# awslabs/flowgger

Measured on NVIDIA H100. Metric: log lines/sec parsed (RFC5424), higher is better.
Workload: dtype u8

## Files before the change

### flowgger_b200/csrc/fg_abi.cu

```cuda
#include <cuda_runtime.h>

#include <algorithm>
#include <chrono>
#include <cstdio>
#include <cstdlib>
#include <cstring>
#include <ctime>
#include <mutex>
#include <new>
#include <string>
#include <utility>
#include <vector>

#include "../../include/flowgger_cuda.h"
#include "fg_kernels.cuh"
#include "fg_status.h"
#include "fg_rfc3164.cuh"
#include "fg_tz.h"

namespace {

const char* kErrorStrings[FG_ST_COUNT] = {};
struct ErrorTableInit {
    ErrorTableInit() {
// ... 301 lines not shown
    int upload(fg_ctx* c, Buf<uint8_t>& blob) {
        bytes.resize(bytes.size() + 16, 0);
        FG_CUDA(c, blob.alloc(bytes.size(), DEV));
        FG_CUDA(c, cudaMemcpy(blob.d, bytes.data(), bytes.size(), cudaMemcpyHostToDevice));
        return FG_OK;
    }
};

int upload_tz(fg_ctx* c) {
    const fg::TzHostTable& H = c->tz_host;
    Packer p;
    const size_t o_hash = p.add(H.hash), o_key = p.add(H.key), o_zone = p.add(H.zone), o_noff = p.add(H.name_off),
                 o_first = p.add(H.first), o_off = p.add(H.off), o_names = p.add(H.names);
    if (int rc = p.upload(c, c->tz_blob)) return rc;
    const uint8_t* b = c->tz_blob.d;
    fg::TzDeviceTable& T = c->tz_dev;
    T = H.view();
    T.hash = (const unsigned long long*)(b + o_hash);
    T.key = (const long long*)(b + o_key);
    T.zone = (const int32_t*)(b + o_zone);
    T.name_off = (const int32_t*)(b + o_noff);
    T.first = (const int32_t*)(b + o_first);
    T.off = (const int32_t*)(b + o_off);
    T.names = b + o_names;
    return FG_OK;
}

int upload_ltsv_config(fg_ctx* c, const fg_config* cfg) {
    std::vector<uint8_t> names, suffix;
    std::vector<int32_t> name_off{0}, types;
    const int ns = (cfg->ltsv_schema_names && cfg->ltsv_schema_types) ? cfg->ltsv_schema_len : 0;
    for (int k = 0; k < ns; ++k) {
        const char* s = cfg->ltsv_schema_names[k];
        names.insert(names.end(), (const uint8_t*)s, (const uint8_t*)s + strlen(s));
        name_off.push_back((int32_t)names.size());
        types.push_back(cfg->ltsv_schema_types[k]);
    }
    fg::LtsvDeviceConfig& L = c->ltsv;
    L.has_schema = (cfg->ltsv_has_schema || ns > 0) ? 1 : 0;
    L.n_schema = ns;
    L.suffix_present = 0;
    L.suffix_off[0] = 0;
    for (int t = 0; t < 5; ++t) {
        const char* s = cfg->ltsv_suffix[t];
        if (t > 0 && s) {
            L.suffix_present |= 1u << t;
            suffix.insert(suffix.end(), (const uint8_t*)s, (const uint8_t*)s + strlen(s));
        }
        L.suffix_off[t + 1] = (int32_t)suffix.size();
    }
    Packer p;
    const size_t o_names = p.add(names), o_off = p.add(name_off), o_types = p.add(types), o_suf = p.add(suffix);
    if (int rc = p.upload(c, c->ltsv_blob)) return rc;
    const uint8_t* b = c->ltsv_blob.d;
    L.names = b + o_names;
    L.name_off = (const int32_t*)(b + o_off);
    L.types = (const int32_t*)(b + o_types);
    L.suffix = b + o_suf;
    return FG_OK;
}

int current_year(const fg_ctx* c) {
    if (c->r3164_year != 0) return c->r3164_year;
    const time_t now = time(nullptr);
    struct tm g;
    gmtime_r(&now, &g);
    return g.tm_year + 1900;
}

int ensure_format(fg_ctx* c, int fmt) {
    const size_t L = (size_t)c->max_lines;
    if (fmt == FG_FMT_RFC5424) {
        if (!c->rows5.d) {
            FG_CUDA(c, c->rows5.alloc(L, BOTH));
            FG_CUDA(c, c->esc_list.alloc(L, DEV));
            FG_CUDA(c, c->wide_list.alloc(L, DEV));
        }
    } else if (!c->rows.d) {
        FG_CUDA(c, c->rows.alloc(col_off(c, C_COUNT), BOTH));
    }
    if (fmt == FG_FMT_GELF && !c->wide_list.d) FG_CUDA(c, c->wide_list.alloc(L, DEV));
    for (const TableUse& u : kFormatTables[fmt]) {
        const size_t first = u.div ? std::max<size_t>(c->max_bytes / u.div, u.floor) : u.floor;
        const size_t cap = c->tab[u.table].cap;
        if (u.grow ? cap < first : !cap)
            if (int rc = grow_table(c, u.table, first)) return rc;
    }
    if (fmt == FG_FMT_RFC3164) {
        if (!c->tz_host.loaded) {
            std::string err;
            if (!fg::tz_load_dir(c->tzdir.empty() ? nullptr : c->tzdir.c_str(), c->tz_host, err)) return fail(c, FG_E_ARG, err.c_str());
        }
        if (!c->tz_blob.d)
            if (int rc = upload_tz(c)) return rc;
    }
    if (fmt == FG_FMT_LTSV || fmt == FG_FMT_GELF) {
        const size_t need = (fmt == FG_FMT_LTSV ? c->max_bytes / 2 + L : c->max_bytes / 3) + 64;
        if (c->tmp_meta.n < need) {
            c->tmp_name.reset(); c->tmp_val.reset(); c->tmp_meta.reset();
            FG_CUDA(c, c->tmp_name.alloc(need, DEV));
            FG_CUDA(c, c->tmp_val.alloc(need, DEV));
            FG_CUDA(c, c->tmp_meta.alloc(need, DEV));
        }
    }
    return FG_OK;
}

int begin_call(fg_ctx* c, fg_format fmt) {
    if ((int)fmt < 0 || (int)fmt > 3) return fail(c, FG_E_ARG, "unknown format");
    FG_CUDA(c, cudaSetDevice(c->device));
    if (int rc = ensure_format(c, (int)fmt)) return rc;
    c->call_year = current_year(c);
    return FG_OK;
}

int pick_tile(const fg_ctx* c, size_t total_bytes, int n, int fmt) {
    const double mean = n > 0 ? (double)total_bytes / n : 0.0;
    const long lines = fg::lines_per_cta(fmt), gran = 8 * lines;
    const int max_tile[4] = {c->max_tile5, fg::kLtsvMaxTile, fg::kGelfMaxTile, fg::kR3164MaxTile};
    long t = (long)(mean * lines * 1.02) + gran;
    t = (t + gran - 1) / gran * gran;
    t = std::max(t, 8L * 1024);
    t = std::min(t, (long)max_tile[fmt]);
    return (int)t;
}

int launch_lines(fg_ctx* c, int fmt, int line0, int n, int tile, const uint8_t* invalid, int strip_eol, cudaStream_t s,
                 bool time_dominant = false) {
    if (fmt == FG_FMT_RFC5424) {
        fg::Parse5424Params P;
        P.bytes = c->bytes.d;
        P.offsets = c->offsets.d + line0;
        P.n = n;
        P.tile_bytes = tile;
        P.rows = reinterpret_cast<uint4*>(c->rows5.d + line0);
        P.entries = dev<unsigned long long>(c, T_E8);
        P.entry_cap = cap32(c, T_E8);
        P.counters = c->k.d;
        P.esc_list = c->esc_list.d;
        P.wide_list = c->wide_list.d;
        P.arena = dev<uint8_t>(c, T_ARENA);
        P.arena_cap = cap32(c, T_ARENA);
        P.wide_rows = dev<fg::WideRow>(c, T_WIDE);
        P.wide_cap = cap32(c, T_WIDE);
        P.wentry_name = dev<int2>(c, T_ENTRIES, 0);
        P.wentry_val = dev<unsigned long long>(c, T_ENTRIES, 1);
        P.wentry_meta = dev<uint8_t>(c, T_ENTRIES, 2);
        P.wentry_cap = cap32(c, T_ENTRIES);
        P.line0 = line0;
        P.bad_offsets = c->k.d + fg::K5_BAD_OFFSETS;
        P.line_invalid = invalid;
        P.strip_eol = strip_eol;
        P.num_sms = c->num_sms;
        FG_CUDA(c, cudaMemsetAsync(c->k.d + fg::K5_ESC_LIST, 0, 8, s));
        FG_CUDA(c, fg::launch_parse5424(P, s, time_dominant ? c->ev_dom0.h : nullptr, time_dominant ? c->ev_dom1.h : nullptr));
        c->launches += 2;
        return FG_OK;
    }
    fg::ParseParams P;
    P.bytes = c->bytes.d;
    P.offsets = c->offsets.d + line0;
    P.n = n;
    P.line0 = line0;
    P.tile_bytes = tile;
    P.num_sms = c->num_sms;
    uint8_t* r = c->rows.d;
    P.ts = (double*)(r + col_off(c, C_TS)) + line0;
    P.meta = (uint32_t*)(r + col_off(c, C_META)) + line0;
    P.host = (int2*)(r + col_off(c, C_HOST)) + line0;
    P.app = (int2*)(r + col_off(c, C_APP)) + line0;
    P.proc = (int2*)(r + col_off(c, C_PROC)) + line0;
    P.msgid = (int2*)(r + col_off(c, C_MSGID)) + line0;
    P.msg = (int2*)(r + col_off(c, C_MSG)) + line0;
    P.full = (int2*)(r + col_off(c, C_FULL)) + line0;
    P.sd = (int2*)(r + col_off(c, C_SD)) + line0;
    P.entry_name = dev<int2>(c, T_ENTRIES, 0);
    P.entry_val = dev<unsigned long long>(c, T_ENTRIES, 1);
    P.entry_meta = dev<uint8_t>(c, T_ENTRIES, 2);
    P.tmp_name = c->tmp_name.d;
    P.tmp_val = c->tmp_val.d;
    P.tmp_meta = c->tmp_meta.d;
    P.line_invalid = invalid;
    P.strip_eol = strip_eol;
    P.entry_counter = c->k.d + fg::K5_ENTRIES;
    P.entry_cap = cap32(c, T_ENTRIES);
    P.bad_offsets = c->k.d + fg::K5_BAD_OFFSETS;
    P.slow_list = c->wide_list.d;
    P.slow_count = c->k.d + fg::K5_WIDE_LIST;
    if (fmt == FG_FMT_GELF) FG_CUDA(c, cudaMemsetAsync(c->k.d + fg::K5_WIDE_LIST, 0, 4, s));
    P.ltsv = c->ltsv;
    P.r3164.year = c->call_year;
    P.r3164.tz = c->tz_dev;
    P.r3164.arena = dev<uint8_t>(c, T_ARENA);
    P.r3164.arena_cap = cap32(c, T_ARENA);
    P.r3164.arena_counter = c->k.d + fg::K5_ARENA;
    if (time_dominant) FG_CUDA(c, cudaEventRecord(c->ev_dom0, s));
    FG_CUDA(c, fg::launch_parse(fmt, P, s));
    if (time_dominant) FG_CUDA(c, cudaEventRecord(c->ev_dom1, s));
    c->launches += fmt == FG_FMT_GELF ? 2 : 1;
    return FG_OK;
}

bool gelf_fusable(int fmt) { return fmt == FG_FMT_RFC5424 || fmt == FG_FMT_RFC3164; }

int launch_encode(fg_ctx* c, int fmt, int k, int l0, int n, int tile, cudaStream_t s) {
    fg::GelfEncodeParams E{};
    E.bytes = c->bytes.d;
    E.offsets = c->offsets.d + l0;
    E.n = n;
    if (fmt == FG_FMT_RFC5424) {
        E.rows = reinterpret_cast<const uint4*>(c->rows5.d + l0);
    } else {
        const uint8_t* r = c->rows.d;
        E.r3_ts = (const double*)(r + col_off(c, C_TS)) + l0;
        E.r3_meta = (const uint32_t*)(r + col_off(c, C_META)) + l0;
        E.r3_host = (const int2*)(r + col_off(c, C_HOST)) + l0;
        E.r3_msg = (const int2*)(r + col_off(c, C_MSG)) + l0;
        E.r3_full = (const int2*)(r + col_off(c, C_FULL)) + l0;
    }
    E.entries = dev<unsigned long long>(c, T_E8);
    E.arena = dev<uint8_t>(c, T_ARENA);
    E.wide_rows = dev<fg::WideRow>(c, T_WIDE);
    E.wentry_name = dev<int2>(c, T_ENTRIES, 0);
    E.wentry_val = dev<unsigned long long>(c, T_ENTRIES, 1);
    E.wentry_meta = dev<uint8_t>(c, T_ENTRIES, 2);
    E.static_blob = c->static_blob.d;
    E.n_static = c->n_static;
    E.static_key_off = c->d_static_key_off;
    E.static_lit_off = c->d_static_lit_off;
    E.static_kind = c->d_static_kind;
    E.lens = c->enc_lens.d + l0;
    E.rel = c->enc_rel.d + l0;
    E.base = c->enc_base.d + k;
    E.out = c->enc_out.d;
    E.out_cap = c->enc_out_cap;
    E.out_offsets = c->enc_offsets.d + l0;
    E.status = c->enc_status.d + l0;
    E.bad_offsets = c->k.d + fg::K5_BAD_OFFSETS;
    E.entry_cap = cap32(c, T_E8);
    E.wide_cap = cap32(c, T_WIDE);
    E.wentry_cap = cap32(c, T_ENTRIES);
    E.arena_cap = cap32(c, T_ARENA);
    E.tile_bytes = std::min(4 * tile, c->max_tile5);
    FG_CUDA(c, fg::launch_gelf_encode(fmt, E, c->scan_temp.d, c->scan_temp_bytes, s));
    c->launches += 4;
    return FG_OK;
}

bool col_used(int col) { return !(col == C_APP || col == C_PROC || col == C_MSGID); }

void fill_out(fg_ctx* c, int fmt, int n, const uint32_t* tot, fg_batch_out* out) {
    out->n = n;
    for (const TableUse& u : kFormatTables[fmt]) {
        const uint32_t rows = u.counter >= 0 ? tot[u.counter] : 0;
        switch (u.table) {
            case T_ENTRIES:
                out->entry_name = host<fg_span>(c, T_ENTRIES, 0);
                out->entry_val = host<uint64_t>(c, T_ENTRIES, 1);
                out->entry_meta = host<uint8_t>(c, T_ENTRIES, 2);
                out->n_entries = (int32_t)rows;
                break;
            case T_E8:
                out->entries8 = host<uint64_t>(c, T_E8);
                out->n_entries8 = (int32_t)rows;
                break;
            case T_ARENA:
                out->arena = host<uint8_t>(c, T_ARENA);
                out->arena_bytes = (int64_t)rows;
                break;
            case T_WIDE:
                out->wide_rows = host<fg_wide_row>(c, T_WIDE);
                out->n_wide = (int32_t)rows;
                break;
        }
    }
    if (fmt == FG_FMT_RFC5424) {
        out->rows5424 = c->rows5.h;
        return;
    }
    uint8_t* r = c->rows.h;
    out->ts = (const double*)(r + col_off(c, C_TS));
    out->meta = (const uint32_t*)(r + col_off(c, C_META));
    out->hostname = (const fg_span*)(r + col_off(c, C_HOST));
    out->msg = (const fg_span*)(r + col_off(c, C_MSG));
    out->full_msg = (const fg_span*)(r + col_off(c, C_FULL));
    out->sd = (const fg_span*)(r + col_off(c, C_SD));
}

int copy_rows_d2h(fg_ctx* c, int fmt, int line0, int n, cudaStream_t s) {
    if (n <= 0) return FG_OK;
    if (fmt == FG_FMT_RFC5424) {
        FG_CUDA(c, cudaMemcpyAsync(c->rows5.h + line0, c->rows5.d + line0, (size_t)n * 32, cudaMemcpyDeviceToHost, s));
        return FG_OK;
    }
    for (int col = C_TS; col <= C_META; ++col) {
        const size_t o = col_off(c, col) + (size_t)line0 * kColW[col];
        FG_CUDA(c, cudaMemcpyAsync(c->rows.h + o, c->rows.d + o, (size_t)n * kColW[col], cudaMemcpyDeviceToHost, s));
    }
    const size_t pitch = (size_t)c->max_lines * 8;
    int col = C_HOST;
    while (col < C_COUNT) {
        if (!col_used(col)) { ++col; continue; }
        int end = col;
        while (end + 1 < C_COUNT && col_used(end + 1)) ++end;
        const size_t o = col_off(c, col) + (size_t)line0 * 8;
        FG_CUDA(c, cudaMemcpy2DAsync(c->rows.h + o, pitch, c->rows.d + o, pitch, (size_t)n * 8, (size_t)(end - col + 1),
                                     cudaMemcpyDeviceToHost, s));
// ... 762 lines not shown
```

### flowgger_b200/csrc/fg_kernels.cuh

```cuda
#pragma once
#include <stdint.h>
#ifdef FG_HOST_EMU
#include "../../tests/emu/cuda_shim.h"
#else
#include <cuda_runtime.h>
#endif

namespace fg {

struct LtsvDeviceConfig {
    int32_t has_schema;
    int32_t n_schema;
    const uint8_t* names;
    const int32_t* name_off;
    const int32_t* types;
    const uint8_t* suffix;
    int32_t suffix_off[6];
    uint32_t suffix_present;
};

struct TzDeviceTable {
    int32_t n_names;
    int32_t min_len, max_len;
    uint32_t first_mask[8];
    const unsigned long long* hash;
    const int32_t* zone;
    const int32_t* name_off;
    const uint8_t* names;
    const int32_t* first;
    const long long* key;
    const int32_t* off;
};
struct R3164DeviceConfig {
    int32_t year;
    TzDeviceTable tz;
    uint8_t* arena;
    uint32_t arena_cap;
    uint32_t* arena_counter;
};

struct ParseParams {
    const uint8_t* bytes;
    const int32_t* offsets;
    int32_t n;
    int32_t line0;
    int32_t tile_bytes;
    double* ts;
    uint32_t* meta;
    int2* host;
    int2* app;
    int2* proc;
    int2* msgid;
    int2* msg;
    int2* full;
    int2* sd;
    int2* entry_name;
    unsigned long long* entry_val;
    uint8_t* entry_meta;
    int2* tmp_name;
    unsigned long long* tmp_val;
    uint8_t* tmp_meta;
    const uint8_t* line_invalid;
    int32_t strip_eol;
    uint32_t* entry_counter;
    uint32_t entry_cap;
    const uint32_t* bad_offsets;
    uint32_t* slow_list;
    uint32_t* slow_count;
    int32_t num_sms;
    LtsvDeviceConfig ltsv;
    R3164DeviceConfig r3164;
};

struct Row5424 {
    double ts;
    uint32_t meta;
    uint32_t sd_first;
    uint16_t sd_count;
    uint16_t sp[5];
    uint16_t msg_off, msg_len;
};
static_assert(sizeof(Row5424) == 32, "Row5424 must be 32 bytes");
struct WideRow {
    int32_t line;
    uint32_t meta;
    double ts;
    int2 host, app, proc, msgid, msg, full, sd;
};
static_assert(sizeof(WideRow) == 72, "WideRow must be 72 bytes");

enum { K5_ENTRIES = 0, K5_ARENA = 1, K5_WIDE_ROWS = 2, K5_WIDE_ENTRIES = 3, K5_ESC_LIST = 4, K5_WIDE_LIST = 5, K5_BAD_OFFSETS = 6,
       K5_COUNT = 8 };

struct Parse5424Params {
    const uint8_t* bytes;
    const int32_t* offsets;
    int32_t n;
    int32_t tile_bytes;
    uint4* rows;
    unsigned long long* entries;
    uint32_t entry_cap;
    uint32_t* counters;
    uint32_t* esc_list;
    uint32_t* wide_list;
    uint8_t* arena;
    uint32_t arena_cap;
    WideRow* wide_rows;
    uint32_t wide_cap;
    int2* wentry_name;
    unsigned long long* wentry_val;
    uint8_t* wentry_meta;
    uint32_t wentry_cap;
    int32_t line0;
    const uint32_t* bad_offsets;
    const uint8_t* line_invalid;
    int32_t strip_eol;
    int32_t num_sms;
};

cudaError_t launch_parse5424(const Parse5424Params& p, cudaStream_t stream, cudaEvent_t dom0 = nullptr, cudaEvent_t dom1 = nullptr);
cudaError_t configure_parse5424(int max_tile_bytes);
int parse5424_smem_bytes(int tile_bytes);

struct GelfEncodeParams {
    const uint8_t* bytes;
    const int32_t* offsets;
    int32_t n;
    const uint4* rows;
    const unsigned long long* entries;
    const uint8_t* arena;
    const WideRow* wide_rows;
    const int2* wentry_name;
    const unsigned long long* wentry_val;
    const uint8_t* wentry_meta;
    const uint8_t* static_blob;
    int32_t n_static;
    const int32_t* static_key_off;
    const int32_t* static_lit_off;
    const int32_t* static_kind;
    unsigned long long* lens;
    unsigned long long* rel;
    unsigned long long* base;
    uint8_t* out;
    unsigned long long out_cap;
    long long* out_offsets;
    uint8_t* status;
    const uint32_t* bad_offsets;
    uint32_t entry_cap, wide_cap, wentry_cap;
    int32_t tile_bytes;
    const double* r3_ts;
    const uint32_t* r3_meta;
    const int2* r3_host;
    const int2* r3_msg;
    const int2* r3_full;
    uint32_t arena_cap;
};
cudaError_t configure_gelf_encode(int max_tile_bytes);
cudaError_t launch_gelf_encode(int fmt, const GelfEncodeParams& p, void* d_scan_temp, size_t scan_temp_bytes, cudaStream_t stream);
size_t gelf_scan_temp_bytes(int n);

#ifndef FG_R5_LINES
#define FG_R5_LINES 64
#endif
#ifndef FG_R5_MINB
#define FG_R5_MINB 16
#endif
constexpr int kRfc5424LinesPerCta = FG_R5_LINES;
constexpr int kRfc5424CtasPerSm = FG_R5_MINB;
#ifndef FG_LTSV_LINES
#define FG_LTSV_LINES 64
#endif
#ifndef FG_LTSV_THREADS
#define FG_LTSV_THREADS 256
#endif
constexpr int kLtsvLinesPerCta = FG_LTSV_LINES;
constexpr int kLtsvThreadsPerCta = FG_LTSV_THREADS;
constexpr int kLtsvStageSlots = kLtsvLinesPerCta * 24;
constexpr int kLtsvMaxTile = 65024;
#ifndef FG_GELF_LINES
#define FG_GELF_LINES 64
#endif
#ifndef FG_GELF_THREADS
#define FG_GELF_THREADS 256
#endif
constexpr int kGelfLinesPerCta = FG_GELF_LINES;
constexpr int kGelfThreadsPerCta = FG_GELF_THREADS;
constexpr int kGelfCtasPerSm = 3;
constexpr int kGelfStageSlots = kGelfLinesPerCta * 16;
constexpr int kGelfMaxTile = 65024;
#ifndef FG_R3_LINES
#define FG_R3_LINES 64
#endif
#ifndef FG_R3_MINB
#define FG_R3_MINB 16
#endif
#ifndef FG_R3_LOCKSTEP
#define FG_R3_LOCKSTEP 1
#endif
constexpr int kR3164LinesPerCta = FG_R3_LINES;
constexpr int kR3164CtasPerSm = FG_R3_MINB;
constexpr int kR3164MaxTile = 65024;
constexpr int lines_per_cta(int fmt) {
    return fmt == 0 ? kRfc5424LinesPerCta : (fmt == 1 ? kLtsvLinesPerCta : (fmt == 2 ? kGelfLinesPerCta : kR3164LinesPerCta));
}

cudaError_t launch_parse(int fmt, const ParseParams& p, cudaStream_t stream);
cudaError_t launch_parse_ltsv(const ParseParams& p, cudaStream_t stream);
cudaError_t configure_parse_ltsv(int max_tile_bytes);
int parse_ltsv_smem_bytes(int tile_bytes, bool typed);
cudaError_t launch_parse_gelf(const ParseParams& p, cudaStream_t stream);
cudaError_t configure_parse_gelf(int max_tile_bytes);
int parse_gelf_smem_bytes(int tile_bytes);
cudaError_t launch_parse3164(const ParseParams& p, cudaStream_t stream);
cudaError_t configure_parse3164(int max_tile_bytes);
cudaError_t launch_check_offsets(const int32_t* d_offsets, int n, long long max_bytes, uint32_t* d_flag, cudaStream_t stream);
cudaError_t configure_kernels(int max_tile5424);
const char* kernel_build_info();

cudaError_t launch_split_chunk(const uint8_t* d_bytes, long long nbytes, long long c0, long long c1, int is_last, uint32_t* d_seg,
                               uint32_t* d_run, int32_t* d_cum_k, int32_t* d_offsets, int32_t* d_n_lines, int max_lines,
                               uint8_t* d_invalid, int delim, cudaStream_t stream);
int split_segments(long long nbytes);

}
```

### flowgger_b200/csrc/fg_parse5424.cu

```cuda
#include "fg_kernels.cuh"

#include "fg_common.cuh"
#include "fg_r5fast.cuh"
#include "fg_rfc5424.cuh"
#include "fg_status.h"
#include "fg_tma.cuh"

namespace fg {

namespace {

constexpr int kFastLines = kRfc5424LinesPerCta;
constexpr int kFastCtasPerSm = kRfc5424CtasPerSm;

template <int LINES, int MINB>
__global__ void __launch_bounds__(LINES, MINB) parse5424_kernel(const __grid_constant__ Parse5424Params P) {
    extern __shared__ __align__(128) uint8_t tile[];
    __shared__ __align__(8) uint64_t mbar;
    __shared__ uint32_t scan_ws[2 * (LINES / 32)];
    __shared__ uint32_t s_base[3];

    const int tid = threadIdx.x;
    const uint32_t lane = (uint32_t)tid & 31u;
    const int first = blockIdx.x * LINES;
    const int last = min(P.n, first + LINES);
    uint32_t* bmI = reinterpret_cast<uint32_t*>(tile + P.tile_bytes);
    if (*P.bad_offsets) return;
    if (tid == 0) mbar_init(&mbar, 1);
    __syncthreads();

    uint32_t parity = 0;
    int cur = first;
    while (cur < last) {
        const int i = cur + tid;
        const int o0 = __ldg(P.offsets + min(i, last));
        const int o1 = __ldg(P.offsets + min(i + 1, last));
        const int ocur = __ldg(P.offsets + cur);
        const int base = ocur & ~15;
        const bool fits = (i < last) && (o1 - base <= P.tile_bytes);
        const int r = __syncthreads_count(fits);
        if (r == 0) {
            if (tid == 0) P.wide_list[atomicAdd(P.counters + K5_WIDE_LIST, 1u)] = (uint32_t)cur;
            cur += 1;
            continue;
        }
        const int oend = __ldg(P.offsets + cur + r);
        const uint32_t nbytes = (uint32_t)((oend - base) + 15) & ~15u;
        if (tid == 0) {
            fence_proxy_async();
            mbar_expect_tx(&mbar, nbytes);
            bulk_g2s(tile, P.bytes + base, nbytes, &mbar);
        }
        mbar_wait(&mbar, parity);
        parity ^= 1u;

        const int nword = (int)((nbytes + 31u) >> 5);
        for (int g = tid; g < nword; g += LINES) {
            const uint4 v0 = reinterpret_cast<const uint4*>(tile)[2 * g], v1 = reinterpret_cast<const uint4*>(tile)[2 * g + 1];
            bmI[g] = r5_classify16(v0.x, v0.y, v0.z, v0.w) | (r5_classify16(v1.x, v1.y, v1.z, v1.w) << 16);
        }
        if (tid < 3) bmI[nword + tid] = 0;
        __syncthreads();

        const bool active = tid < r;
        int ls = active ? o0 - base : 0;
        int le = active ? o1 - base : 0;
        bool bad_utf8 = false;
        if (P.strip_eol && le > ls) {
            if (P.strip_eol == 2) {
                if (tile[le - 1] == 0) --le;
            } else if (tile[le - 1] == '\n') {
                --le;
                if (le > ls && tile[le - 1] == '\r') --le;
            }
            if (P.line_invalid != nullptr && P.line_invalid[i]) bad_utf8 = true;
        }
        const bool too_long = le - ls > 65535;
        R5Fast res;
        const bool regular = r5_regular(tile, bmI, ls, (too_long || bad_utf8 || !active) ? ls : le, res);
        if (bad_utf8) {
            res.status = FG_ES_INVALID_UTF8;
            res.n_entries = 0;
        }
        const bool wide = active && !regular && !bad_utf8;
        const uint32_t my_n = (active && !wide && res.status == FG_ST_OK) ? res.n_entries : 0u;
        const bool esc = my_n != 0u && res.esc;

        uint32_t xa = my_n, xb = (esc ? 1u : 0u) | (wide ? 0x100u : 0u);
#pragma unroll
        for (int d = 1; d < 32; d <<= 1) {
            const uint32_t ya = __shfl_up_sync(0xFFFFFFFFu, xa, d), yb = __shfl_up_sync(0xFFFFFFFFu, xb, d);
            if (lane >= (uint32_t)d) { xa += ya; xb += yb; }
        }
        const int wid = tid >> 5;
        constexpr int kWarps = LINES / 32;
        if (lane == 31u) { scan_ws[wid] = xa; scan_ws[kWarps + wid] = xb; }
        __syncthreads();
        uint32_t before_a = 0, before_b = 0, total = 0, total_b = 0;
#pragma unroll
        for (int w = 0; w < kWarps; ++w) {
            const uint32_t ta = scan_ws[w], tb = scan_ws[kWarps + w];
            if (w < wid) { before_a += ta; before_b += tb; }
            total += ta;
            total_b += tb;
        }
        const uint32_t excl = before_a + xa - my_n;
        const uint32_t pos_b = before_b + xb - ((esc ? 1u : 0u) | (wide ? 0x100u : 0u));
        const uint32_t n_esc = total_b & 0xFFu, n_wide = total_b >> 8;
        if (total | total_b) {
            if (tid == 0 && total) s_base[0] = atomicAdd(P.counters + K5_ENTRIES, total);
            if (tid == 32 % LINES && n_esc) s_base[1] = atomicAdd(P.counters + K5_ESC_LIST, n_esc);
            if (tid == 33 % LINES && n_wide) s_base[2] = atomicAdd(P.counters + K5_WIDE_LIST, n_wide);
            __syncthreads();
        }
        const uint32_t esc_at = pos_b & 0xFFu, wide_at = pos_b >> 8;
        uint32_t my_begin = 0;
        if (my_n) {
            my_begin = s_base[0] + excl;
            if ((unsigned long long)my_begin + my_n <= (unsigned long long)P.entry_cap) {
                unsigned long long* dst = P.entries + my_begin;
                for (uint32_t k = 0; k < my_n; ++k) dst[k] = res.stage[k];
            }
        }
        if (esc) P.esc_list[s_base[1] + esc_at] = (uint32_t)i;
        if (wide) P.wide_list[s_base[2] + wide_at] = (uint32_t)i;
        if (active && !wide) {
            const bool ok = res.status == FG_ST_OK;
            const uint32_t meta = ok ? (res.facility << 8) | (res.severity << 16) | (res.flags << 24) : res.status | 0x00FFFF00u;
            uint4 lo4, hi4;
            lo4.x = (uint32_t)__double2loint(res.ts);
            lo4.y = (uint32_t)__double2hiint(res.ts);
            lo4.z = meta;
            lo4.w = my_begin;
            hi4.x = my_n | ((uint32_t)res.sp1 << 16);
            hi4.y = (uint32_t)res.sp2 | ((uint32_t)res.sp3 << 16);
            hi4.z = (uint32_t)res.sp4 | ((uint32_t)res.sp5 << 16);
            hi4.w = (uint32_t)res.msg_o | ((uint32_t)res.msg_l << 16);
            if (!ok) {
                lo4.x = lo4.y = 0u;
                hi4 = make_uint4(0u, 0u, 0u, 0u);
            }
            P.rows[2 * (size_t)i] = lo4;
            P.rows[2 * (size_t)i + 1] = hi4;
        }
        __syncthreads();
        cur += r;
    }
}

__device__ __forceinline__ void unescape_lines(const Parse5424Params& P, uint32_t first_item, uint32_t stride) {
    const uint32_t cnt = P.counters[K5_ESC_LIST];
    const uint32_t lane = threadIdx.x & 31u;
    for (uint32_t j0 = first_item; j0 < cnt; j0 += stride) {
        const uint32_t j = j0 + lane;
        const bool valid = j < cnt;
        uint32_t first = 0, count = 0;
        int o0 = 0;
        if (valid) {
            const uint32_t line = P.esc_list[j];
            const uint4 lo4 = P.rows[2 * (size_t)line], hi4 = P.rows[2 * (size_t)line + 1];
            o0 = P.offsets[line];
            first = lo4.w;
            count = hi4.x & 0xFFFFu;
            if ((unsigned long long)first + count > (unsigned long long)P.entry_cap) count = 0;
        }
        uint32_t need = 0;
        for (uint32_t e = 0; e < count; ++e) {
            const unsigned long long v = P.entries[first + e];
            if (!(v & kE8Header) && (v & kE8Esc)) need += (2u + (uint32_t)((v >> 32) & 0xFFFFu) - ((uint32_t)((v >> 16) & 0xFFFFu) + 2u) + 1u) & ~1u;
        }
        uint32_t inc = need;
#pragma unroll
        for (int d = 1; d < 32; d <<= 1) {
            const uint32_t y = __shfl_up_sync(0xFFFFFFFFu, inc, d);
            if (lane >= (uint32_t)d) inc += y;
        }
        const uint32_t warp_total = __shfl_sync(0xFFFFFFFFu, inc, 31);
        uint32_t abase = 0;
        if (lane == 0 && warp_total) abase = atomicAdd(P.counters + K5_ARENA, warp_total);
        abase = __shfl_sync(0xFFFFFFFFu, abase, 0);
        if ((unsigned long long)abase + warp_total > (unsigned long long)P.arena_cap) continue;
        uint32_t at = abase + inc - need;
        uint32_t e = 0;
        for (;;) {
            unsigned long long v = 0;
            bool have = false;
            for (; e < count; ++e) {
                v = P.entries[first + e];
                if (!(v & kE8Header) && (v & kE8Esc)) { have = true; break; }
            }
            if (!__any_sync(0xFFFFFFFFu, have)) break;
            const int ne = (int)((v >> 16) & 0xFFFFu), ve = (int)((v >> 32) & 0xFFFFu);
            const int len = have ? ve - (ne + 2) : 0;
            const uint8_t* src = P.bytes + o0 + ne + 2;
            uint8_t* dst = P.arena + at + 2;
            int k = 0, o = 0;
            while (__any_sync(0xFFFFFFFFu, k < len)) {
                if (k < len) {
                    const uint32_t c = src[k++];
                    if (c != '\\') {
                        dst[o++] = (uint8_t)c;
                    } else if (k < len) {
                        const uint32_t d = src[k++];
                        if (d != '"' && d != '\\' && d != ']') dst[o++] = '\\';
                        dst[o++] = (uint8_t)d;
                    }
                }
            }
            if (have) {
                *reinterpret_cast<uint16_t*>(P.arena + at) = (uint16_t)o;
                P.entries[first + e] = (v & 0xFFFFFFFFull) | ((unsigned long long)(at >> 1) << 32) | kE8Arena;
                at += (2u + (uint32_t)len + 1u) & ~1u;
                ++e;
            }
        }
    }
}

__device__ __forceinline__ void wide_lines(const Parse5424Params& P, int (*marks)[32], uint32_t first_item, uint32_t stride) {
    const uint32_t cnt = P.counters[K5_WIDE_LIST];
    const uint32_t lane = threadIdx.x & 31u;
    const EntrySink sink = {P.wentry_name, P.wentry_val, P.wentry_meta};
    for (uint32_t j0 = first_item; j0 < cnt; j0 += stride) {
        const uint32_t j = j0 + lane;
        const bool valid = j < cnt;
        uint32_t line = 0;
        int o0 = 0, len = 0;
        bool bad_utf8 = false;
        if (valid) {
            line = P.wide_list[j];
            o0 = P.offsets[line];
            len = P.offsets[line + 1] - o0;
            if (P.strip_eol && len > 0) {
                if (P.strip_eol == 2) {
                    if (P.bytes[o0 + len - 1] == 0) --len;
                } else if (P.bytes[o0 + len - 1] == '\n') {
                    --len;
                    if (len > 0 && P.bytes[o0 + len - 1] == '\r') --len;
                }
                if (P.line_invalid != nullptr && P.line_invalid[line]) bad_utf8 = true;
            }
            if (bad_utf8) len = 0;
        }
        LineResult res;
        rfc5424_parse_line<32>(P.bytes + o0, len, o0, &marks[0][lane], res, sink, 0u, false);
        uint32_t n = (valid && !bad_utf8 && res.status == FG_ST_OK) ? res.n_entries : 0u;
        uint32_t wbase = 0;
        if (n) {
            wbase = atomicAdd(P.counters + K5_WIDE_ENTRIES, n);
            if ((unsigned long long)wbase + n > (unsigned long long)P.wentry_cap) n = 0;
        }
        {
            LineResult again;
            rfc5424_parse_line<32>(P.bytes + o0, n ? len : 0, o0, &marks[0][lane], again, sink, wbase, true);
        }
        if (!valid) continue;
        for (uint32_t k = 0; k < n; ++k) {
            const uint32_t e = wbase + k;
            const uint8_t m = sink.meta[e];
            if ((m & 0x07u) == 0u && (m & 0x08u)) {
                const unsigned long long v = sink.val[e];
                const uint32_t off = (uint32_t)v, l = (uint32_t)(v >> 32);
                const uint32_t ul = (uint32_t)r5_unescape(P.bytes + off, (int)l, nullptr);
                const uint32_t at = atomicAdd(P.counters + K5_ARENA, (ul + 1u) & ~1u);
                if ((unsigned long long)at + ul <= (unsigned long long)P.arena_cap) r5_unescape(P.bytes + off, (int)l, P.arena + at);
                sink.val[e] = (unsigned long long)at | ((unsigned long long)ul << 32);
                sink.meta[e] = (uint8_t)0x80u;
            }
        }
        if (bad_utf8) {
            res.status = FG_ES_INVALID_UTF8;
            res.flags = 0;
            res.facility = res.severity = 0xFFu;
        }
        const bool ok = res.status == FG_ST_OK;
        if (!ok) {
            P.rows[2 * (size_t)line] = make_uint4(0u, 0u, res.status | 0x00FFFF00u, 0u);
            P.rows[2 * (size_t)line + 1] = make_uint4(0u, 0u, 0u, 0u);
            continue;
        }
        const uint32_t widx = atomicAdd(P.counters + K5_WIDE_ROWS, 1u);
        const uint32_t meta = res.status | (res.facility << 8) | (res.severity << 16) | ((res.flags | kFlagWide) << 24);
        if (widx < P.wide_cap) {
            WideRow w;
            w.line = P.line0 + (int32_t)line;
            w.meta = meta;
            w.ts = res.ts;
            w.host = make_int2(ok ? o0 + res.host_o : -1, res.host_l);
            w.app = make_int2(ok ? o0 + res.app_o : -1, res.app_l);
            w.proc = make_int2(ok ? o0 + res.proc_o : -1, res.proc_l);
            w.msgid = make_int2(ok ? o0 + res.mid_o : -1, res.mid_l);
            w.msg = make_int2(ok && res.msg_o >= 0 ? o0 + res.msg_o : -1, res.msg_l);
            w.full = make_int2(ok && res.full_o >= 0 ? o0 + res.full_o : -1, res.full_l);
            w.sd = make_int2((int)wbase, (int)(ok ? n : 0u));
            P.wide_rows[widx] = w;
        }
        P.rows[2 * (size_t)line] = make_uint4((uint32_t)__double2loint(res.ts), (uint32_t)__double2hiint(res.ts), meta, widx);
        P.rows[2 * (size_t)line + 1] = make_uint4(0u, 0u, 0u, 0u);
    }
}

__global__ void __launch_bounds__(128) post5424_kernel(const __grid_constant__ Parse5424Params P, int esc_ctas) {
    __shared__ int marks[4][6][32];
    if (*P.bad_offsets) return;
    const uint32_t warp = threadIdx.x >> 5;
    if ((int)blockIdx.x < esc_ctas) {
        unescape_lines(P, (blockIdx.x * 4u + warp) * 32u, (uint32_t)esc_ctas * 128u);
    } else {
        const uint32_t wctas = gridDim.x - (uint32_t)esc_ctas;
        wide_lines(P, marks[warp], ((blockIdx.x - (uint32_t)esc_ctas) * 4u + warp) * 32u, wctas * 128u);
    }
}

}

int parse5424_smem_bytes(int tile_bytes) { return tile_bytes + tile_bytes / 8 + 16; }

cudaError_t configure_parse5424(int max_tile_bytes) {
    return cudaFuncSetAttribute(parse5424_kernel<kFastLines, kFastCtasPerSm>, cudaFuncAttributeMaxDynamicSharedMemorySize,
                                parse5424_smem_bytes(max_tile_bytes));
}

cudaError_t launch_parse5424(const Parse5424Params& p, cudaStream_t stream, cudaEvent_t dom0, cudaEvent_t dom1) {
    if (p.n <= 0) return cudaSuccess;
    const int grid = (p.n + kFastLines - 1) / kFastLines;
    if (dom0) cudaEventRecord(dom0, stream);
    parse5424_kernel<kFastLines, kFastCtasPerSm><<<grid, kFastLines, parse5424_smem_bytes(p.tile_bytes), stream>>>(p);
    if (dom1) cudaEventRecord(dom1, stream);
    const long long sms = p.num_sms;
    const int esc_ctas = (int)min((long long)(p.n + 127) / 128, sms * 12);
    const int wide_ctas = (int)min((long long)(p.n + 127) / 128, sms * 4);
    post5424_kernel<<<esc_ctas + wide_ctas, 128, 0, stream>>>(p, esc_ctas);
    return cudaGetLastError();
}

}
```

Baseline: 6.713 billion.

## Rework RFC5424 post-pass with dynamic work queue and warp-cooperative unescaping

The post kernel now uses a persistent grid sized from occupancy, where warps pull 32-item chunks from an atomic counter covering both wide lines and escaped lines, replacing the fixed split between escape and wide CTAs. Unescaping is rewritten so the warp gathers escaped entries into a shared queue and processes their raw bytes cooperatively, one byte per lane, with ballot-based backslash handling, instead of one thread per line looping serially. The aim is to fix load imbalance and divergence when few lines carry escapes. The cost is a per-chunk global atomic, extra shared memory, and a more intricate byte-level unescape that could hold correctness bugs.

```diff
diff --git a/flowgger_b200/csrc/fg_abi.cu b/flowgger_b200/csrc/fg_abi.cu
--- a/flowgger_b200/csrc/fg_abi.cu
+++ b/flowgger_b200/csrc/fg_abi.cu
@@ -477,7 +477,7 @@
         P.line_invalid = invalid;
         P.strip_eol = strip_eol;
         P.num_sms = c->num_sms;
-        FG_CUDA(c, cudaMemsetAsync(c->k.d + fg::K5_ESC_LIST, 0, 8, s));
+        FG_CUDA(c, cudaMemsetAsync(c->k.d + fg::K5_ESC_LIST, 0, sizeof(uint32_t) * (fg::K5_POST_NEXT + 1 - fg::K5_ESC_LIST), s));
         FG_CUDA(c, fg::launch_parse5424(P, s, time_dominant ? c->ev_dom0.h : nullptr, time_dominant ? c->ev_dom1.h : nullptr));
         c->launches += 2;
         return FG_OK;
diff --git a/flowgger_b200/csrc/fg_kernels.cuh b/flowgger_b200/csrc/fg_kernels.cuh
--- a/flowgger_b200/csrc/fg_kernels.cuh
+++ b/flowgger_b200/csrc/fg_kernels.cuh
@@ -89,8 +89,8 @@
 };
 static_assert(sizeof(WideRow) == 72, "WideRow must be 72 bytes");
 
-enum { K5_ENTRIES = 0, K5_ARENA = 1, K5_WIDE_ROWS = 2, K5_WIDE_ENTRIES = 3, K5_ESC_LIST = 4, K5_WIDE_LIST = 5, K5_BAD_OFFSETS = 6,
-       K5_COUNT = 8 };
+enum { K5_ENTRIES = 0, K5_ARENA = 1, K5_WIDE_ROWS = 2, K5_WIDE_ENTRIES = 3, K5_ESC_LIST = 4, K5_WIDE_LIST = 5, K5_POST_NEXT = 6,
+       K5_BAD_OFFSETS = 7, K5_COUNT = 8 };
 
 struct Parse5424Params {
     const uint8_t* bytes;
diff --git a/flowgger_b200/csrc/fg_parse5424.cu b/flowgger_b200/csrc/fg_parse5424.cu
--- a/flowgger_b200/csrc/fg_parse5424.cu
+++ b/flowgger_b200/csrc/fg_parse5424.cu
@@ -1,4 +1,6 @@
 #include "fg_kernels.cuh"
+
+#include <atomic>
 
 #include "fg_common.cuh"
 #include "fg_r5fast.cuh"
@@ -148,177 +150,258 @@
     }
 }
 
-__device__ __forceinline__ void unescape_lines(const Parse5424Params& P, uint32_t first_item, uint32_t stride) {
-    const uint32_t cnt = P.counters[K5_ESC_LIST];
+constexpr int kPostWarps = 4;
+constexpr int kEscQueue = 64;
+
+struct EscQueue {
+    uint32_t cum[kEscQueue + 1];
+    uint32_t src[kEscQueue];
+    uint32_t dst[kEscQueue];
+    uint32_t ent[kEscQueue];
+    uint32_t lo[kEscQueue];
+};
+
+__device__ __forceinline__ uint32_t esc_value_at(const EscQueue& q, uint32_t nq, uint32_t pos) {
+    uint32_t v = 0;
+#pragma unroll
+    for (uint32_t step = kEscQueue / 2; step; step >>= 1)
+        if (v + step < nq && q.cum[v + step] <= pos) v += step;
+    return v;
+}
+
+__device__ void flush_escaped(const Parse5424Params& P, EscQueue& q, uint32_t nq, uint32_t raw, uint32_t need) {
     const uint32_t lane = threadIdx.x & 31u;
-    for (uint32_t j0 = first_item; j0 < cnt; j0 += stride) {
-        const uint32_t j = j0 + lane;
-        const bool valid = j < cnt;
-        uint32_t first = 0, count = 0;
-        int o0 = 0;
-        if (valid) {
-            const uint32_t line = P.esc_list[j];
-            const uint4 lo4 = P.rows[2 * (size_t)line], hi4 = P.rows[2 * (size_t)line + 1];
-            o0 = P.offsets[line];
-            first = lo4.w;
-            count = hi4.x & 0xFFFFu;
-            if ((unsigned long long)first + count > (unsigned long long)P.entry_cap) count = 0;
-        }
-        uint32_t need = 0;
-        for (uint32_t e = 0; e < count; ++e) {
-            const unsigned long long v = P.entries[first + e];
-            if (!(v & kE8Header) && (v & kE8Esc)) need += (2u + (uint32_t)((v >> 32) & 0xFFFFu) - ((uint32_t)((v >> 16) & 0xFFFFu) + 2u) + 1u) & ~1u;
-        }
-        uint32_t inc = need;
+    uint32_t abase = 0;
+    if (lane == 0) {
+        abase = atomicAdd(P.counters + K5_ARENA, need);
+        q.cum[nq] = raw;
+    }
+    abase = __shfl_sync(0xFFFFFFFFu, abase, 0);
+    __syncwarp();
+    if ((unsigned long long)abase + need <= (unsigned long long)P.arena_cap) {
+        const uint32_t upto = 0xFFFFFFFFu >> (31u - lane);
+        uint32_t v = 0, c = 0;
+        if (lane < raw) {
+            v = esc_value_at(q, nq, lane);
+            c = P.bytes[q.src[v] + lane - q.cum[v]];
+        }
+        uint32_t carry_run = 0, carry_kept = 0;
+        for (uint32_t s = 0; s < raw; s += 32u) {
+            const uint32_t pos = s + lane, cv = v, cc = c;
+            const bool valid = pos < raw;
+            if (pos + 32u < raw) {
+                v = esc_value_at(q, nq, pos + 32u);
+                c = P.bytes[q.src[v] + pos + 32u - q.cum[v]];
+            }
+            const uint32_t next0 = __shfl_sync(0xFFFFFFFFu, c, 0);
+            uint32_t nx = __shfl_down_sync(0xFFFFFFFFu, cc, 1);
+            if (lane == 31u) nx = next0;
+            const bool last = valid && pos + 1u == q.cum[cv + 1u];
+            const bool bs = valid && cc == '\\';
+            const uint32_t nb = ~__ballot_sync(0xFFFFFFFFu, bs) & upto;
+            const uint32_t st = __ballot_sync(0xFFFFFFFFu, valid && pos == q.cum[cv]) & upto;
+            int rs = -(int)carry_run;
+            if (nb) rs = 32 - __clz(nb);
+            const int vs = st ? 31 - __clz(st) : 0;
+            if (st) rs = max(rs, vs);
+            const bool drop = bs && (((int)lane - rs) & 1) == 0 && (last || nx == '"' || nx == '\\' || nx == ']');
+            const bool keep = valid && !drop;
+            const uint32_t kept = __popc(__ballot_sync(0xFFFFFFFFu, keep) & (upto >> 1) & ~((1u << vs) - 1u)) + (st ? 0u : carry_kept);
+            const uint32_t at = abase + q.dst[cv];
+            if (keep) P.arena[at + 2u + kept] = (uint8_t)cc;
+            if (last) {
+                *reinterpret_cast<uint16_t*>(P.arena + at) = (uint16_t)(kept + (keep ? 1u : 0u));
+                P.entries[q.ent[cv]] = (unsigned long long)q.lo[cv] | ((unsigned long long)(at >> 1) << 32) | kE8Arena;
+            }
+            carry_run = __shfl_sync(0xFFFFFFFFu, bs ? (uint32_t)((int)lane - rs + 1) & 1u : 0u, 31);
+            carry_kept = __shfl_sync(0xFFFFFFFFu, kept + (keep ? 1u : 0u), 31);
+        }
+    }
+    __syncwarp();
+}
+
+__device__ __forceinline__ void unescape_lines(const Parse5424Params& P, EscQueue& q, uint32_t j0, uint32_t j1) {
+    const uint32_t lane = threadIdx.x & 31u;
+    const uint32_t j = j0 + lane;
+    uint32_t first = 0, count = 0, o0 = 0;
+    if (j < j1) {
+        const uint32_t line = P.esc_list[j];
+        first = P.rows[2 * (size_t)line].w;
+        count = P.rows[2 * (size_t)line + 1].x & 0xFFFFu;
+        o0 = (uint32_t)P.offsets[line];
+        if ((unsigned long long)first + count > (unsigned long long)P.entry_cap) count = 0;
+    }
+    uint32_t incl = count;
+#pragma unroll
+    for (int d = 1; d < 32; d <<= 1) {
+        const uint32_t y = __shfl_up_sync(0xFFFFFFFFu, incl, d);
+        if (lane >= (uint32_t)d) incl += y;
+    }
+    const uint32_t total = __shfl_sync(0xFFFFFFFFu, incl, 31);
+    auto row_at = [&](uint32_t r0, uint32_t& e, uint32_t& lo0) -> unsigned long long {
+        const uint32_t r = r0 + lane;
+        uint32_t k = 0;
+#pragma unroll
+        for (uint32_t step = 16; step; step >>= 1) {
+            const uint32_t t = __shfl_sync(0xFFFFFFFFu, incl, k + step - 1u);
+            if (t <= r) k += step;
+        }
+        k = min(k, 31u);
+        const uint32_t kfirst = __shfl_sync(0xFFFFFFFFu, first, k), kcount = __shfl_sync(0xFFFFFFFFu, count, k);
+        const uint32_t kincl = __shfl_sync(0xFFFFFFFFu, incl, k);
+        lo0 = __shfl_sync(0xFFFFFFFFu, o0, k);
+        e = kfirst + r - (kincl - kcount);
+        return r < total ? P.entries[e] : 0ull;
+    };
+    uint32_t nq = 0, raw = 0, need = 0;
+    uint32_t next_e = 0, next_o0 = 0;
+    unsigned long long next_v = total ? row_at(0, next_e, next_o0) : 0ull;
+    for (uint32_t r0 = 0; r0 < total; r0 += 32u) {
+        const uint32_t e = next_e, ko0 = next_o0;
+        const unsigned long long v = next_v;
+        if (r0 + 32u < total) next_v = row_at(r0 + 32u, next_e, next_o0);
+        const bool esc = !(v & kE8Header) && (v & kE8Esc);
+        const uint32_t ne = (uint32_t)(v >> 16) & 0xFFFFu;
+        const uint32_t len = esc ? ((uint32_t)(v >> 32) & 0xFFFFu) - (ne + 2u) : 0u;
+        const uint32_t rec = esc ? (2u + len + 1u) & ~1u : 0u;
+        const uint32_t m = __ballot_sync(0xFFFFFFFFu, esc);
+        if (!m) continue;
+        if (nq + __popc(m) > (uint32_t)kEscQueue) {
+            flush_escaped(P, q, nq, raw, need);
+            nq = raw = need = 0;
+        }
+        uint32_t xr = len, xn = rec;
 #pragma unroll
         for (int d = 1; d < 32; d <<= 1) {
-            const uint32_t y = __shfl_up_sync(0xFFFFFFFFu, inc, d);
-            if (lane >= (uint32_t)d) inc += y;
-        }
-        const uint32_t warp_total = __shfl_sync(0xFFFFFFFFu, inc, 31);
-        uint32_t abase = 0;
-        if (lane == 0 && warp_total) abase = atomicAdd(P.counters + K5_ARENA, warp_total);
-        abase = __shfl_sync(0xFFFFFFFFu, abase, 0);
-        if ((unsigned long long)abase + warp_total > (unsigned long long)P.arena_cap) continue;
-        uint32_t at = abase + inc - need;
-        uint32_t e = 0;
-        for (;;) {
-            unsigned long long v = 0;
-            bool have = false;
-            for (; e < count; ++e) {
-                v = P.entries[first + e];
-                if (!(v & kE8Header) && (v & kE8Esc)) { have = true; break; }
-            }
-            if (!__any_sync(0xFFFFFFFFu, have)) break;
-            const int ne = (int)((v >> 16) & 0xFFFFu), ve = (int)((v >> 32) & 0xFFFFu);
-            const int len = have ? ve - (ne + 2) : 0;
-            const uint8_t* src = P.bytes + o0 + ne + 2;
-            uint8_t* dst = P.arena + at + 2;
-            int k = 0, o = 0;
-            while (__any_sync(0xFFFFFFFFu, k < len)) {
-                if (k < len) {
-                    const uint32_t c = src[k++];
-                    if (c != '\\') {
-                        dst[o++] = (uint8_t)c;
-                    } else if (k < len) {
-                        const uint32_t d = src[k++];
-                        if (d != '"' && d != '\\' && d != ']') dst[o++] = '\\';
-                        dst[o++] = (uint8_t)d;
-                    }
-                }
-            }
-            if (have) {
-                *reinterpret_cast<uint16_t*>(P.arena + at) = (uint16_t)o;
-                P.entries[first + e] = (v & 0xFFFFFFFFull) | ((unsigned long long)(at >> 1) << 32) | kE8Arena;
-                at += (2u + (uint32_t)len + 1u) & ~1u;
-                ++e;
-            }
-        }
-    }
-}
-
-__device__ __forceinline__ void wide_lines(const Parse5424Params& P, int (*marks)[32], uint32_t first_item, uint32_t stride) {
-    const uint32_t cnt = P.counters[K5_WIDE_LIST];
+            const uint32_t yr = __shfl_up_sync(0xFFFFFFFFu, xr, d), yn = __shfl_up_sync(0xFFFFFFFFu, xn, d);
+            if (lane >= (uint32_t)d) { xr += yr; xn += yn; }
+        }
+        if (esc) {
+            const uint32_t at = nq + __popc(m & ((1u << lane) - 1u));
+            q.cum[at] = raw + xr - len;
+            q.dst[at] = need + xn - rec;
+            q.src[at] = ko0 + ne + 2u;
+            q.ent[at] = e;
+            q.lo[at] = (uint32_t)v;
+        }
+        nq += __popc(m);
+        raw += __shfl_sync(0xFFFFFFFFu, xr, 31);
+        need += __shfl_sync(0xFFFFFFFFu, xn, 31);
+        __syncwarp();
+    }
+    if (nq) flush_escaped(P, q, nq, raw, need);
+}
+
+__device__ __forceinline__ void wide_lines(const Parse5424Params& P, int (*marks)[32], uint32_t j0, uint32_t cnt) {
     const uint32_t lane = threadIdx.x & 31u;
     const EntrySink sink = {P.wentry_name, P.wentry_val, P.wentry_meta};
-    for (uint32_t j0 = first_item; j0 < cnt; j0 += stride) {
-        const uint32_t j = j0 + lane;
-        const bool valid = j < cnt;
-        uint32_t line = 0;
-        int o0 = 0, len = 0;
-        bool bad_utf8 = false;
-        if (valid) {
-            line = P.wide_list[j];
-            o0 = P.offsets[line];
-            len = P.offsets[line + 1] - o0;
-            if (P.strip_eol && len > 0) {
-                if (P.strip_eol == 2) {
-                    if (P.bytes[o0 + len - 1] == 0) --len;
-                } else if (P.bytes[o0 + len - 1] == '\n') {
-                    --len;
-                    if (len > 0 && P.bytes[o0 + len - 1] == '\r') --len;
-                }
-                if (P.line_invalid != nullptr && P.line_invalid[line]) bad_utf8 = true;
-            }
-            if (bad_utf8) len = 0;
-        }
-        LineResult res;
-        rfc5424_parse_line<32>(P.bytes + o0, len, o0, &marks[0][lane], res, sink, 0u, false);
-        uint32_t n = (valid && !bad_utf8 && res.status == FG_ST_OK) ? res.n_entries : 0u;
-        uint32_t wbase = 0;
-        if (n) {
-            wbase = atomicAdd(P.counters + K5_WIDE_ENTRIES, n);
-            if ((unsigned long long)wbase + n > (unsigned long long)P.wentry_cap) n = 0;
-        }
-        {
-            LineResult again;
-            rfc5424_parse_line<32>(P.bytes + o0, n ? len : 0, o0, &marks[0][lane], again, sink, wbase, true);
-        }
-        if (!valid) continue;
-        for (uint32_t k = 0; k < n; ++k) {
-            const uint32_t e = wbase + k;
-            const uint8_t m = sink.meta[e];
-            if ((m & 0x07u) == 0u && (m & 0x08u)) {
-                const unsigned long long v = sink.val[e];
-                const uint32_t off = (uint32_t)v, l = (uint32_t)(v >> 32);
-                const uint32_t ul = (uint32_t)r5_unescape(P.bytes + off, (int)l, nullptr);
-                const uint32_t at = atomicAdd(P.counters + K5_ARENA, (ul + 1u) & ~1u);
-                if ((unsigned long long)at + ul <= (unsigned long long)P.arena_cap) r5_unescape(P.bytes + off, (int)l, P.arena + at);
-                sink.val[e] = (unsigned long long)at | ((unsigned long long)ul << 32);
-                sink.meta[e] = (uint8_t)0x80u;
-            }
-        }
-        if (bad_utf8) {
-            res.status = FG_ES_INVALID_UTF8;
-            res.flags = 0;
-            res.facility = res.severity = 0xFFu;
-        }
-        const bool ok = res.status == FG_ST_OK;
-        if (!ok) {
-            P.rows[2 * (size_t)line] = make_uint4(0u, 0u, res.status | 0x00FFFF00u, 0u);
-            P.rows[2 * (size_t)line + 1] = make_uint4(0u, 0u, 0u, 0u);
-            continue;
-        }
-        const uint32_t widx = atomicAdd(P.counters + K5_WIDE_ROWS, 1u);
-        const uint32_t meta = res.status | (res.facility << 8) | (res.severity << 16) | ((res.flags | kFlagWide) << 24);
-        if (widx < P.wide_cap) {
-            WideRow w;
-            w.line = P.line0 + (int32_t)line;
-            w.meta = meta;
-            w.ts = res.ts;
-            w.host = make_int2(ok ? o0 + res.host_o : -1, res.host_l);
-            w.app = make_int2(ok ? o0 + res.app_o : -1, res.app_l);
-            w.proc = make_int2(ok ? o0 + res.proc_o : -1, res.proc_l);
-            w.msgid = make_int2(ok ? o0 + res.mid_o : -1, res.mid_l);
-            w.msg = make_int2(ok && res.msg_o >= 0 ? o0 + res.msg_o : -1, res.msg_l);
-            w.full = make_int2(ok && res.full_o >= 0 ? o0 + res.full_o : -1, res.full_l);
-            w.sd = make_int2((int)wbase, (int)(ok ? n : 0u));
-            P.wide_rows[widx] = w;
-        }
-        P.rows[2 * (size_t)line] = make_uint4((uint32_t)__double2loint(res.ts), (uint32_t)__double2hiint(res.ts), meta, widx);
+    const uint32_t j = j0 + lane;
+    const bool valid = j < cnt;
+    uint32_t line = 0;
+    int o0 = 0, len = 0;
+    bool bad_utf8 = false;
+    if (valid) {
+        line = P.wide_list[j];
+        o0 = P.offsets[line];
+        len = P.offsets[line + 1] - o0;
+        if (P.strip_eol && len > 0) {
+            if (P.strip_eol == 2) {
+                if (P.bytes[o0 + len - 1] == 0) --len;
+            } else if (P.bytes[o0 + len - 1] == '\n') {
+                --len;
+                if (len > 0 && P.bytes[o0 + len - 1] == '\r') --len;
+            }
+            if (P.line_invalid != nullptr && P.line_invalid[line]) bad_utf8 = true;
+        }
+        if (bad_utf8) len = 0;
+    }
+    LineResult res;
+    rfc5424_parse_line<32>(P.bytes + o0, len, o0, &marks[0][lane], res, sink, 0u, false);
+    uint32_t n = (valid && !bad_utf8 && res.status == FG_ST_OK) ? res.n_entries : 0u;
+    uint32_t wbase = 0;
+    if (n) {
+        wbase = atomicAdd(P.counters + K5_WIDE_ENTRIES, n);
+        if ((unsigned long long)wbase + n > (unsigned long long)P.wentry_cap) n = 0;
+    }
+    {
+        LineResult again;
+        rfc5424_parse_line<32>(P.bytes + o0, n ? len : 0, o0, &marks[0][lane], again, sink, wbase, true);
+    }
+    if (!valid) return;
+    for (uint32_t k = 0; k < n; ++k) {
+        const uint32_t e = wbase + k;
+        const uint8_t m = sink.meta[e];
+        if ((m & 0x07u) == 0u && (m & 0x08u)) {
+            const unsigned long long v = sink.val[e];
+            const uint32_t off = (uint32_t)v, l = (uint32_t)(v >> 32);
+            const uint32_t ul = (uint32_t)r5_unescape(P.bytes + off, (int)l, nullptr);
+            const uint32_t at = atomicAdd(P.counters + K5_ARENA, (ul + 1u) & ~1u);
+            if ((unsigned long long)at + ul <= (unsigned long long)P.arena_cap) r5_unescape(P.bytes + off, (int)l, P.arena + at);
+            sink.val[e] = (unsigned long long)at | ((unsigned long long)ul << 32);
+            sink.meta[e] = (uint8_t)0x80u;
+        }
+    }
+    if (bad_utf8) {
+        res.status = FG_ES_INVALID_UTF8;
+        res.flags = 0;
+        res.facility = res.severity = 0xFFu;
+    }
+    const bool ok = res.status == FG_ST_OK;
+    if (!ok) {
+        P.rows[2 * (size_t)line] = make_uint4(0u, 0u, res.status | 0x00FFFF00u, 0u);
         P.rows[2 * (size_t)line + 1] = make_uint4(0u, 0u, 0u, 0u);
-    }
-}
-
-__global__ void __launch_bounds__(128) post5424_kernel(const __grid_constant__ Parse5424Params P, int esc_ctas) {
-    __shared__ int marks[4][6][32];
+        return;
+    }
+    const uint32_t widx = atomicAdd(P.counters + K5_WIDE_ROWS, 1u);
+    const uint32_t meta = res.status | (res.facility << 8) | (res.severity << 16) | ((res.flags | kFlagWide) << 24);
+    if (widx < P.wide_cap) {
+        WideRow w;
+        w.line = P.line0 + (int32_t)line;
+        w.meta = meta;
+        w.ts = res.ts;
+        w.host = make_int2(ok ? o0 + res.host_o : -1, res.host_l);
+        w.app = make_int2(ok ? o0 + res.app_o : -1, res.app_l);
+        w.proc = make_int2(ok ? o0 + res.proc_o : -1, res.proc_l);
+        w.msgid = make_int2(ok ? o0 + res.mid_o : -1, res.mid_l);
+        w.msg = make_int2(ok && res.msg_o >= 0 ? o0 + res.msg_o : -1, res.msg_l);
+        w.full = make_int2(ok && res.full_o >= 0 ? o0 + res.full_o : -1, res.full_l);
+        w.sd = make_int2((int)wbase, (int)(ok ? n : 0u));
+        P.wide_rows[widx] = w;
+    }
+    P.rows[2 * (size_t)line] = make_uint4((uint32_t)__double2loint(res.ts), (uint32_t)__double2hiint(res.ts), meta, widx);
+    P.rows[2 * (size_t)line + 1] = make_uint4(0u, 0u, 0u, 0u);
+}
+
+__global__ void __launch_bounds__(kPostWarps * 32) post5424_kernel(const __grid_constant__ Parse5424Params P) {
+    __shared__ int marks[kPostWarps][6][32];
+    __shared__ EscQueue queue[kPostWarps];
     if (*P.bad_offsets) return;
-    const uint32_t warp = threadIdx.x >> 5;
-    if ((int)blockIdx.x < esc_ctas) {
-        unescape_lines(P, (blockIdx.x * 4u + warp) * 32u, (uint32_t)esc_ctas * 128u);
-    } else {
-        const uint32_t wctas = gridDim.x - (uint32_t)esc_ctas;
-        wide_lines(P, marks[warp], ((blockIdx.x - (uint32_t)esc_ctas) * 4u + warp) * 32u, wctas * 128u);
-    }
-}
+    const uint32_t warp = threadIdx.x >> 5, lane = threadIdx.x & 31u;
+    const uint32_t n_wide = P.counters[K5_WIDE_LIST], n = n_wide + P.counters[K5_ESC_LIST];
+    for (;;) {
+        uint32_t b = 0;
+        if (lane == 0) b = atomicAdd(P.counters + K5_POST_NEXT, 32u);
+        b = __shfl_sync(0xFFFFFFFFu, b, 0);
+        if (b >= n) break;
+        if (b < n_wide) wide_lines(P, marks[warp], b, n_wide);
+        if (b + 32u > n_wide) unescape_lines(P, queue[warp], max(b, n_wide) - n_wide, min(b + 32u, n) - n_wide);
+    }
+}
+
+std::atomic<int> g_post_ctas_per_sm{0};
 
 }
 
 int parse5424_smem_bytes(int tile_bytes) { return tile_bytes + tile_bytes / 8 + 16; }
 
 cudaError_t configure_parse5424(int max_tile_bytes) {
-    return cudaFuncSetAttribute(parse5424_kernel<kFastLines, kFastCtasPerSm>, cudaFuncAttributeMaxDynamicSharedMemorySize,
-                                parse5424_smem_bytes(max_tile_bytes));
+    cudaError_t e = cudaFuncSetAttribute(parse5424_kernel<kFastLines, kFastCtasPerSm>, cudaFuncAttributeMaxDynamicSharedMemorySize,
+                                         parse5424_smem_bytes(max_tile_bytes));
+    if (e != cudaSuccess) return e;
+    int ctas = 0;
+    e = cudaOccupancyMaxActiveBlocksPerMultiprocessor(&ctas, post5424_kernel, kPostWarps * 32, 0);
+    if (e == cudaSuccess) g_post_ctas_per_sm.store(ctas, std::memory_order_relaxed);
+    return e;
 }
 
 cudaError_t launch_parse5424(const Parse5424Params& p, cudaStream_t stream, cudaEvent_t dom0, cudaEvent_t dom1) {
@@ -327,10 +410,9 @@
     if (dom0) cudaEventRecord(dom0, stream);
     parse5424_kernel<kFastLines, kFastCtasPerSm><<<grid, kFastLines, parse5424_smem_bytes(p.tile_bytes), stream>>>(p);
     if (dom1) cudaEventRecord(dom1, stream);
-    const long long sms = p.num_sms;
-    const int esc_ctas = (int)min((long long)(p.n + 127) / 128, sms * 12);
-    const int wide_ctas = (int)min((long long)(p.n + 127) / 128, sms * 4);
-    post5424_kernel<<<esc_ctas + wide_ctas, 128, 0, stream>>>(p, esc_ctas);
+    const long long per_wave = (long long)p.num_sms * max(g_post_ctas_per_sm.load(std::memory_order_relaxed), 1);
+    const int post_ctas = (int)min((long long)(p.n + kPostWarps * 32 - 1) / (kPostWarps * 32), per_wave);
+    post5424_kernel<<<post_ctas, kPostWarps * 32, 0, stream>>>(p);
     return cudaGetLastError();
 }
 
```

New measurement: 6.952 billion (median of 6 runs). 1.04x the previous value.
